# cocowy1/Cost-Volume-Aggregation-in-Stereo-Matching-Revisited

Measured on AMD Instinct MI355X. Metric: cost-volumes/sec (fwd+bwd) at 544x960 D=192, higher is better.
Workload: dtype f32

## Files before the change

### cost-volume-aggregation-in-stereo-matching-revisited_amd/csrc/conv3d_wgrad_f16x2.hip

```cpp
#include "dca_frag.h"
#include "dca_tiles.h"
#include <type_traits>

namespace {

constexpr int NT = 2;
constexpr int TD = 2, TH = 4, TW = 16;
constexpr int NROW = TD * TH;
constexpr int NGRP = 2, NACC = 7;
static_assert(NROW / NGRP == TH, "a K-step group is one d plane of the tile");
constexpr int HD = TD + 2, HH = TH + 2, NHROW = HD * HH;
constexpr int XV = TW + 2;
constexpr int VB = 64;
constexpr int X_TERM = NHROW * XV * VB;
constexpr int Y_TERM = NROW * TW * VB;
constexpr int X_OFF = 0, Y_OFF = NT * X_TERM;
constexpr int IMG_BYTES = Y_OFF + NT * Y_TERM;
constexpr int LDS_BYTES = 2 * IMG_BYTES;
static_assert(LDS_BYTES >= 4 * 7 * 4096 && LDS_BYTES + 128 <= 160 * 1024, "LDS");
constexpr int NXW = NT * NHROW * XV * 4, KXW = (NXW + 511) / 512;
constexpr int NYW = NT * NROW * TW * 4, KYW = NYW / 512;
constexpr int NXQ = NHROW * 4 * 4, NXE = NHROW * 2 * 4, NYQ = NROW * 4 * 4;
static_assert(NXQ + NYQ == 512 && NYW % 512 == 0, "staging items");

struct WX2Args {
  const float* x;
  const float* dy;
  float* part;
  int N, Cx, Cy, D, H, W;
  int nTD, nTH, nTW, nCxT;
  const int* xexps;
  const int* yexps;
};

template <bool XP, bool YP>
__global__ __launch_bounds__(512) void wgrad3_f16x2_kernel(WX2Args a) {
  extern __shared__ __attribute__((aligned(16))) char smem[];
  const int tid = threadIdx.x, lane = tid & 63, wv = tid >> 6, l31 = lane & 31, half = lane >> 5;
  const int grp = wv >> 2, wq = wv & 3;
  const int ct = blockIdx.y, cy0 = (ct / a.nCxT) * 32, cx0 = (ct % a.nCxT) * 32;

  const DcaTileWalk walk = dca_my_tile_walk((long)a.N * a.nTD * a.nTH * a.nTW);
  const int t_begin = walk.begin, t_end = walk.end, t_step = walk.step;

  f32x16 acc[NACC];
#pragma unroll
  for (int j = 0; j < NACC; ++j)
#pragma unroll
    for (int r = 0; r < 16; ++r) acc[j][r] = 0.f;

  const int cstride = a.D * a.H * a.W;
  const long xsample = (long)a.Cx * cstride, ysample = (long)a.Cy * cstride;

  const int lane_off = (8 * half + ((lane & 15) >> 2)) * VB + (16 * ((lane >> 4) & 1) + 4 * (lane & 3)) * 2;

  float4 pw[(XP ? KXW : 0) + (YP ? KYW : 0) + ((XP || YP) ? 0 : 1)];
  float4 rq[(XP && YP) ? 1 : 8];
  float re[XP ? 1 : 8];
  int ex8[(XP && YP) ? 1 : 8];
  if constexpr (!XP || !YP) {
    const bool isy = !YP && (XP || tid >= NXQ);
#pragma unroll
    for (int j = 0; j < 8; ++j) {
      const int c = (isy ? cy0 : cx0) + (tid & 3) * 8 + j;
      ex8[j] = (c < (isy ? a.Cy : a.Cx)) ? dca_coherent_loadi((isy ? a.yexps : a.xexps) + c) : 0;
    }
  }
  int xcrd[XP ? KXW : 1], ycrd[YP ? KYW : 1];
  if constexpr (XP) {
#pragma unroll
    for (int k = 0; k < KXW; ++k) {
      const int it = tid + 512 * k, cg = it & 3, vv = it >> 2, v = vv % XV, r = vv / XV, hrow = r % NHROW, term = r / NHROW;
      xcrd[k] = (it < NXW) ? ((hrow / HH) | ((hrow % HH) << 4) | (v << 8) | (term << 16) | (cg << 20)) : -1;
    }
  }
  if constexpr (YP) {
#pragma unroll
    for (int k = 0; k < KYW; ++k) {
      const int it = tid + 512 * k, cg = it & 3, vv = it >> 2, v = vv % TW, r = vv / TW, row = r % NROW, term = r / NROW;
      ycrd[k] = (row / TH) | ((row % TH) << 4) | (v << 8) | (term << 16) | (cg << 20);
    }
  }
  auto decode = [&](int tile, int& n, int& d0, int& h0, int& w0) __attribute__((always_inline)) {
    dca_tile_decode<TD, TH, TW>(tile, a.nTD, a.nTH, a.nTW, n, d0, h0, w0);
  };
  auto load_tile = [&](int n, int d0, int h0, int w0, int part = -1) __attribute__((always_inline)) {
    const __amdgpu_buffer_rsrc_t xr = dca_rsrc(a.x + (long)n * xsample, xsample * 4);
    const __amdgpu_buffer_rsrc_t yr = dca_rsrc(a.dy + (long)n * ysample, ysample * 4);
    if constexpr (XP) {
#pragma unroll
      for (int k = 0; k < KXW; ++k) {
        if ((part == 0 && k >= 4) || (part == 1 && k < 4)) continue;
        int crd = xcrd[k];
        asm volatile("" : "+v"(crd));
        const int d = d0 - 1 + (crd & 15), h = h0 - 1 + ((crd >> 4) & 15), w = w0 - 1 + ((crd >> 8) & 255);
        const int term = (crd >> 16) & 1, g = (cx0 >> 3) + ((crd >> 20) & 3);
        const int ok = (int)(crd >= 0) & (int)(g * 8 < a.Cx) & (int)((unsigned)d < (unsigned)a.D) &
                       (int)((unsigned)h < (unsigned)a.H) & (int)((unsigned)w < (unsigned)a.W);
        pw[k] = dca_bload4(xr, term * (a.Cx * cstride * 2) + (g * cstride + (d * a.H + h) * a.W + w) * 16, ok);
      }
    } else {
      if (part != 1 && tid < NXQ) {
        const int cg = tid & 3, quad = (tid >> 2) & 3, hrow = tid >> 4;
        const int d = d0 - 1 + hrow / HH, h = h0 - 1 + hrow % HH, w = w0 + 4 * quad, c0 = cx0 + cg * 8;
        const int ok = (int)((unsigned)d < (unsigned)a.D) & (int)((unsigned)h < (unsigned)a.H) & (int)(w + 3 < a.W);
        const int off = (c0 * cstride + (d * a.H + h) * a.W + w) * 4;
#pragma unroll
        for (int j = 0; j < 8; ++j) rq[j] = dca_bload4(xr, off + j * cstride * 4, ok & (int)(c0 + j < a.Cx));
      }
      if (part != 0 && tid < NXE) {
        const int cg = tid & 3, side = (tid >> 2) & 1, hrow = tid >> 3;
        const int d = d0 - 1 + hrow / HH, h = h0 - 1 + hrow % HH, w = side ? w0 + TW : w0 - 1, c0 = cx0 + cg * 8;
        const int ok = (int)((unsigned)d < (unsigned)a.D) & (int)((unsigned)h < (unsigned)a.H) & (int)((unsigned)w < (unsigned)a.W);
        const int off = (c0 * cstride + (d * a.H + h) * a.W + w) * 4;
#pragma unroll
        for (int j = 0; j < 8; ++j) re[j] = dca_bload1(xr, off + j * cstride * 4, ok & (int)(c0 + j < a.Cx));
      }
    }
    if (part == 0) return;
    if constexpr (YP) {
#pragma unroll
      for (int k = 0; k < KYW; ++k) {
        int crd = ycrd[k];
        asm volatile("" : "+v"(crd));
        const int d = d0 + (crd & 15), h = h0 + ((crd >> 4) & 15), w = w0 + ((crd >> 8) & 255);
        const int term = (crd >> 16) & 1, g = (cy0 >> 3) + ((crd >> 20) & 3);
        const int ok = (int)(g * 8 < a.Cy) & (int)(d < a.D) & (int)(h < a.H) & (int)(w < a.W);
        pw[(XP ? KXW : 0) + k] = dca_bload4(yr, term * (a.Cy * cstride * 2) + (g * cstride + (d * a.H + h) * a.W + w) * 16, ok);
      }
    } else {
      if (XP || tid >= NXQ) {
        const int u = XP ? tid : tid - NXQ;
        if (u < NYQ) {
          const int cg = u & 3, quad = (u >> 2) & 3, row = u >> 4;
          const int d = d0 + row / TH, h = h0 + row % TH, w = w0 + 4 * quad, c0 = cy0 + cg * 8;
          const int ok = (int)(d < a.D) & (int)(h < a.H) & (int)(w + 3 < a.W);
          const int off = (c0 * cstride + (d * a.H + h) * a.W + w) * 4;
#pragma unroll
          for (int j = 0; j < 8; ++j) rq[j] = dca_bload4(yr, off + j * cstride * 4, ok & (int)(c0 + j < a.Cy));
        }
      }
    }
  };
  typedef __attribute__((address_space(3))) char lds_char;
  const int wvu = __builtin_amdgcn_readfirstlane(tid >> 6);
  const unsigned lds0 = (unsigned)(unsigned long)(lds_char*)smem;
  auto desc = [&](const void* base, long bytes) __attribute__((always_inline)) {
    const unsigned long long b = (unsigned long long)base;
    u32x4 r;
    r.x = __builtin_amdgcn_readfirstlane((unsigned)b);
    r.y = __builtin_amdgcn_readfirstlane((unsigned)(b >> 32)) & 0xffffu;
    r.z = __builtin_amdgcn_readfirstlane((unsigned)bytes);
    r.w = 0x00020000u;
    return r;
  };
  auto glds16 = [&](u32x4 rs, int voff, unsigned lds_byte) __attribute__((always_inline)) {
    unsigned keep;
    asm volatile("s_mov_b32 %0, m0\n\ts_mov_b32 m0, %2\n\ts_nop 0\n\tbuffer_load_dwordx4 %1, %3, 0 offen lds\n\ts_mov_b32 m0, %0"
                 : "=&s"(keep) : "v"(voff), "s"(lds_byte), "s"(rs) : "memory");
  };
  auto glds_tile = [&](int n, int d0, int h0, int w0, int part, int buf) __attribute__((always_inline)) {
    if constexpr (XP && YP) {
      const u32x4 xr = desc(a.x + (long)n * xsample, xsample * 4), yr = desc(a.dy + (long)n * ysample, ysample * 4);
      const unsigned img = lds0 + buf * IMG_BYTES;
#pragma unroll
      for (int k = 0; k < KXW; ++k) {
        if ((part == 0 && k >= 4) || (part == 1 && k < 4)) continue;
        if (512 * k + 64 * wvu < NXW) {
          int crd = xcrd[k];
          asm volatile("" : "+v"(crd));
          const int d = d0 - 1 + (crd & 15), h = h0 - 1 + ((crd >> 4) & 15), w = w0 - 1 + ((crd >> 8) & 255);
          const int term = (crd >> 16) & 1, g = (cx0 >> 3) + ((crd >> 20) & 3);
          const int ok = (int)(g * 8 < a.Cx) & (int)((unsigned)d < (unsigned)a.D) & (int)((unsigned)h < (unsigned)a.H) &
                         (int)((unsigned)w < (unsigned)a.W);
          glds16(xr, dca_pred_off(term * (a.Cx * cstride * 2) + (g * cstride + (d * a.H + h) * a.W + w) * 16, ok),
                 img + X_OFF + (512 * k + 64 * wvu) * 16);
        }
      }
      if (part == 0) return;
#pragma unroll
      for (int k = 0; k < KYW; ++k) {
        int crd = ycrd[k];
        asm volatile("" : "+v"(crd));
        const int d = d0 + (crd & 15), h = h0 + ((crd >> 4) & 15), w = w0 + ((crd >> 8) & 255);
        const int term = (crd >> 16) & 1, g = (cy0 >> 3) + ((crd >> 20) & 3);
        const int ok = (int)(g * 8 < a.Cy) & (int)(d < a.D) & (int)(h < a.H) & (int)(w < a.W);
        glds16(yr, dca_pred_off(term * (a.Cy * cstride * 2) + (g * cstride + (d * a.H + h) * a.W + w) * 16, ok),
               img + Y_OFF + (512 * k + 64 * wvu) * 16);
      }
    }
  };

  auto split_word = [&](const float (&v)[8], char* dst, int term_stride) __attribute__((always_inline)) {
    f16x8 hv, lv;
#pragma unroll
    for (int j = 0; j < 8; ++j) {
      _Float16 h, l;
      x2_split(v[j], ex8[j], h, l);
      hv[j] = h; lv[j] = l;
    }
    *(f16x8*)dst = hv;
    *(f16x8*)(dst + term_stride) = lv;
  };
  auto quad_words = [&](char* dst, int term_stride) __attribute__((always_inline)) {
    const float* q0 = (const float*)&rq[0];
#pragma unroll
    for (int vv = 0; vv < 4; ++vv) {
      const float v[8] = {q0[vv], q0[4 + vv], q0[8 + vv], q0[12 + vv], q0[16 + vv], q0[20 + vv], q0[24 + vv], q0[28 + vv]};
      split_word(v, dst + vv * VB, term_stride);
    }
  };
  auto store_tile = [&]() __attribute__((always_inline)) {
    if constexpr (XP) {
#pragma unroll
      for (int k = 0; k < KXW; ++k) {
        const int it = tid + 512 * k;
        if (it < NXW) *(float4*)(smem + X_OFF + it * 16) = pw[k];
      }
    } else {
      if (tid < NXQ) {
        const int cg = tid & 3, quad = (tid >> 2) & 3, hrow = tid >> 4;
        quad_words(smem + X_OFF + (hrow * XV + 1 + 4 * quad) * VB + cg * 16, X_TERM);
      }
      if (tid < NXE) {
        const int cg = tid & 3, side = (tid >> 2) & 1, hrow = tid >> 3;
        const float v[8] = {re[0], re[1], re[2], re[3], re[4], re[5], re[6], re[7]};
        split_word(v, smem + X_OFF + (hrow * XV + (side ? XV - 1 : 0)) * VB + cg * 16, X_TERM);
      }
    }
    if constexpr (YP) {
#pragma unroll
      for (int k = 0; k < KYW; ++k) *(float4*)(smem + Y_OFF + (tid + 512 * k) * 16) = pw[(XP ? KXW : 0) + k];
    } else {
      if (XP || tid >= NXQ) {
        const int u = XP ? tid : tid - NXQ;
        if (u < NYQ) {
          const int cg = u & 3, quad = (u >> 2) & 3, row = u >> 4;
          quad_words(smem + Y_OFF + (row * TW + 4 * quad) * VB + cg * 16, Y_TERM);
        }
      }
    }
  };

  auto mfma_tile = [&](auto WQC, bool more, int next_tile, int buf) __attribute__((always_inline)) {
    constexpr int WQ = decltype(WQC)::value;
    constexpr int TAP0 = 7 * WQ, TAP1 = (TAP0 + 7 < 27) ? TAP0 + 7 : 27, NTAP = TAP1 - TAP0;
#pragma unroll 1
    for (int i = 0; i < TH; ++i) {
      if ((i == 1 || i == 2) && more) {
        int nn, nd0, nh0, nw0;
        decode(next_tile, nn, nd0, nh0, nw0);
        if constexpr (XP && YP) glds_tile(nn, nd0, nh0, nw0, i - 1, buf ^ 1);
        else load_tile(nn, nd0, nh0, nw0, i - 1);
      }
      const char* yb = smem + buf * IMG_BYTES + Y_OFF + ((grp * TH + i) * TW) * VB + lane_off;
      const char* xb = smem + buf * IMG_BYTES + X_OFF + ((grp * HH + i) * XV) * VB + lane_off;
      f16x8 ay[NT];
#pragma unroll
      for (int term = 0; term < NT; ++term) ay[term] = tr_frag(yb + term * Y_TERM, 4 * VB);
      f16x8 bx[2][NT];
      auto load_b = [&](int tap, int slot) __attribute__((always_inline)) {
        const int kd = tap / 9, kh = (tap / 3) % 3, kw = tap % 3;
#pragma unroll
        for (int term = 0; term < NT; ++term) bx[slot][term] = tr_frag(xb + term * X_TERM + ((kd * HH + kh) * XV + kw) * VB, 4 * VB);
      };
      load_b(TAP0, 0);
#pragma unroll
      for (int j = 0; j < NTAP; ++j) {
        const int cur = j & 1;
        if (j + 1 < NTAP) load_b(TAP0 + j + 1, cur ^ 1);
        acc[j] = __builtin_amdgcn_mfma_f32_32x32x16_f16(ay[0], bx[cur][1], acc[j], 0, 0, 0);
        acc[j] = __builtin_amdgcn_mfma_f32_32x32x16_f16(ay[1], bx[cur][0], acc[j], 0, 0, 0);
        acc[j] = __builtin_amdgcn_mfma_f32_32x32x16_f16(ay[0], bx[cur][0], acc[j], 0, 0, 0);
        if (j + 1 < NTAP) {
          __builtin_amdgcn_sched_group_barrier(0x100, 2, 0);
          __builtin_amdgcn_sched_group_barrier(0x008, 1, 0);
          __builtin_amdgcn_sched_group_barrier(0x100, 2, 0);
          __builtin_amdgcn_sched_group_barrier(0x008, 2, 0);
        }
        __builtin_amdgcn_sched_barrier(0);
      }
    }
  };

  if (t_begin < t_end) {
    int n, d0, h0, w0;
    decode(t_begin, n, d0, h0, w0);
    if constexpr (XP && YP) {
      glds_tile(n, d0, h0, w0, -1, 0);
      __builtin_amdgcn_s_waitcnt(0x0f70);
    } else {
      load_tile(n, d0, h0, w0);
      store_tile();
    }
    __syncthreads();
    int buf = 0;
#pragma unroll 1
    for (int tile = t_begin; tile < t_end; tile += t_step) {
      const bool more = tile + t_step < t_end;
      switch (wq) {
        case 0: mfma_tile(std::integral_constant<int, 0>{}, more, tile + t_step, buf); break;
        case 1: mfma_tile(std::integral_constant<int, 1>{}, more, tile + t_step, buf); break;
        case 2: mfma_tile(std::integral_constant<int, 2>{}, more, tile + t_step, buf); break;
        default: mfma_tile(std::integral_constant<int, 3>{}, more, tile + t_step, buf); break;
      }
      if constexpr (XP && YP) __builtin_amdgcn_s_waitcnt(0x0f70);
      __syncthreads();
      if constexpr (XP && YP) {
        buf ^= 1;
      } else {
        if (more) store_tile();
        __syncthreads();
      }
    }
  }

  __syncthreads();
  int* ey_lds = (int*)(smem + LDS_BYTES);
  if (tid < 32) ey_lds[tid] = (cy0 + tid < a.Cy) ? dca_coherent_loadi(a.yexps + cy0 + tid) : 0;
  __syncthreads();
  const int xe_l = (cx0 + l31 < a.Cx) ? dca_coherent_loadi(a.xexps + cx0 + l31) : 0;
  int ninv[16];
#pragma unroll
  for (int r = 0; r < 16; ++r) ninv[r] = -(ey_lds[(r & 3) + 8 * (r >> 2) + 4 * half] + xe_l);
  float* red = (float*)smem;
  if (grp == 1) {
#pragma unroll
    for (int j = 0; j < 7; ++j)
#pragma unroll
      for (int r = 0; r < 16; ++r)
        red[((wq * 7 + j) * 32 + (r & 3) + 8 * (r >> 2) + 4 * half) * 32 + l31] = acc[j][r];
  }
  __syncthreads();
  if (grp == 0) {
    float* slab = a.part + ((long)blockIdx.x * gridDim.y + ct) * 27 * 1024;
#pragma unroll
    for (int j = 0; j < 7; ++j) {
      const int tap = 7 * wq + j;
      if (tap < 27) {
#pragma unroll
        for (int r = 0; r < 16; ++r) {
          const int co = (r & 3) + 8 * (r >> 2) + 4 * half;
          slab[tap * 1024 + co * 32 + l31] = ldexpf(acc[j][r] + red[((wq * 7 + j) * 32 + co) * 32 + l31], ninv[r]);
        }
      }
    }
  }
}

}

extern "C" long dca_conv3d_wgrad_x2_workspace(int N, int Cx, int Cy, int D, int H, int W) {
  if (N <= 0 || Cx <= 0 || Cy <= 0 || D <= 0 || H <= 0 || W <= 0) return 0;
  return dca_wgrad_split_geometry<TD, TH, TW>(N, Cx, Cy, D, H, W).part_floats;
}

extern "C" int dca_conv3d_wgrad_x2(const void* x, int x_packed, const int* xexps, const void* dy, int dy_packed,
                                   const int* yexps, float* part, float* dw, int N, int Cx, int Cy, int D, int H, int W,
                                   long s_cy, long s_cx, hipStream_t stream) {
  DCA_REQUIRE(x && dy && part && dw && xexps && yexps && N > 0 && Cx > 0 && Cy > 0 && D > 0 && H > 0 && W > 0);
  DCA_REQUIRE(((((uintptr_t)x | (uintptr_t)dy) & 15) == 0));
  DCA_REQUIRE((x_packed ? Cx % 8 == 0 : W % 4 == 0) && (dy_packed ? Cy % 8 == 0 : W % 4 == 0));
  DCA_REQUIRE((long)Cx * D * H * W * 4 < 0x7ffffff0L && (long)Cy * D * H * W * 4 < 0x7ffffff0L);
  WX2Args a;
  a.x = (const float*)x; a.dy = (const float*)dy; a.part = part; a.xexps = xexps; a.yexps = yexps;
  a.N = N; a.Cx = Cx; a.Cy = Cy; a.D = D; a.H = H; a.W = W;
  const DcaWgradSplitGeom g = dca_wgrad_split_geometry<TD, TH, TW>(N, Cx, Cy, D, H, W);
  a.nTD = g.t.nTD; a.nTH = g.t.nTH; a.nTW = g.t.nTW; a.nCxT = g.nCxT;
  DCA_REQUIRE(g.t.fits() && g.nCT <= 65535);
  const int lds = LDS_BYTES + 128;
  auto kern = x_packed ? (dy_packed ? wgrad3_f16x2_kernel<true, true> : wgrad3_f16x2_kernel<true, false>)
                       : (dy_packed ? wgrad3_f16x2_kernel<false, true> : wgrad3_f16x2_kernel<false, false>);
  hipError_t e = hipFuncSetAttribute((const void*)kern, hipFuncAttributeMaxDynamicSharedMemorySize, lds);
  if (e != hipSuccess) return (int)e;
  hipLaunchKernelGGL(kern, dim3(g.nblk, g.nCT), dim3(512), lds, stream, a);
  int st = dca_launch_status();
  if (st) return st;
  return dca_internal_wgrad_reduce(part, dw, g.nblk, g.nCxT, g.nCT, 27, Cy, Cx, s_cy, s_cx, stream);
}
```

### cost-volume-aggregation-in-stereo-matching-revisited_amd/ops.py

```python
from __future__ import annotations

import ctypes
import os
import threading

import torch

from ._call import _C, _L, _chk, _ptr, _raw_device, _raw_stream, _req, _req_no_grad, _stream, _vp
from .guided import GUIDE, guide_params, hints_to_quarter


def _opt(t, name):
    return None if t is None else _req(t, name)


class _GwcVolume(torch.autograd.Function):
    @staticmethod
    def forward(ctx, ref, tgt, maxdisp, num_groups):
        ref, tgt = _req(ref, "build_gwc_volume"), _req(tgt, "build_gwc_volume")
        B, C, H, W = ref.shape
        vol = torch.empty((B, num_groups, maxdisp, H, W), device=ref.device, dtype=torch.float32)
        with torch.cuda.device_of(ref):
            _chk(_L().dca_gwc_volume_fwd(_ptr(ref), _ptr(tgt), _ptr(vol), B, C, H, W, maxdisp, num_groups, _stream()),
                 "dca_gwc_volume_fwd")
# ... 242 lines not shown
        _chk(_L().dca_softargmin_stats(_ptr(x), _ptr(out), B, K, HW, min(radius, K), _stream()), "dca_softargmin_stats")
    return out


class _UpSoftArgmin(torch.autograd.Function):

    @staticmethod
    def forward(ctx, logits, scale):
        logits = _req(logits, "up_softargmin")
        B, n, hc, wc = logits.shape
        disp = torch.empty((B, 1, scale * hc, scale * wc), device=logits.device, dtype=torch.float32)
        with torch.cuda.device_of(logits):
            _chk(_L().dca_up_softargmin_fwd(_ptr(logits), _ptr(disp), B, n, hc, wc, scale, _stream()),
                 "dca_up_softargmin_fwd")
        ctx.save_for_backward(logits)
        ctx.scale = scale
        return disp

    @staticmethod
    def backward(ctx, g):
        (logits,) = ctx.saved_tensors
        g = _req(g, "up_softargmin.backward")
        B, n, hc, wc = logits.shape
        s = ctx.scale
        g1 = torch.empty((B, n, s * hc, s * wc), device=logits.device, dtype=torch.float32)
        gl = torch.empty_like(logits)
        with torch.cuda.device_of(logits):
            _chk(_L().dca_up_softargmin_bwd(_ptr(logits), _ptr(g), _ptr(g1), _ptr(gl), B, n, hc, wc, s, _stream()),
                 "dca_up_softargmin_bwd")
        return gl, None


def up_softargmin(logits, scale):
    if logits.shape[1] > 64 or logits.shape[1] < 2 or scale not in (2, 4, 8):
        return softargmin(trilinear_upsample(logits.unsqueeze(1), scale).squeeze(1))
    return _UpSoftArgmin.apply(logits, int(scale))


def _round_up(a, m):
    return (a + m - 1) // m * m


_CONV_MODE = os.environ.get("DCA_CONV", "x2")
CONV_X3 = _CONV_MODE != "fp32"
CONV_X2 = _CONV_MODE == "x2"
WGRAD_S2_X2 = os.environ.get("DCA_WGRAD_S2", "x2") != "fp32"
DECONV_X3 = os.environ.get("DCA_DECONV", "x3") != "fp32"
C1_WGRAD_FUSED = os.environ.get("DCA_C1_WGRAD", "fused") != "expand"
CONV_S2_X2 = os.environ.get("DCA_CONV_S2", "x2") != "fp32"
BN_FUSE = os.environ.get("DCA_BN_FUSE", "1") != "0"
C1_BWD_FUSE = os.environ.get("DCA_C1_BWD", "fused") != "split"
SKIP_FOLD = os.environ.get("DCA_SKIP_FOLD", "1") != "0"
C1_HEAD_BWD = os.environ.get("DCA_C1_HEAD_BWD", "fused") != "split"
_X3_MIN_WORKGROUPS = 1


AMAX_STATS = {"tagged": 0, "computed": 0, "packed": 0}
CSLOTS = _C["DCA_AMAX_CSLOTS"]
AMAX_EMIT = os.environ.get("DCA_AMAX_EMIT", "1") != "0"
PACK = os.environ.get("DCA_PACK", "1") != "0"


def _cslots(C, device):
    if not AMAX_EMIT:
        return None
    return torch.empty((C * CSLOTS,), device=device, dtype=torch.int32)


def _ver(t):
    return None if t.is_inference() else t._version


def _tag_cmax(t, slots, nslots):
    if slots is not None:
        t._dca_cmax = (slots, int(nslots), _ver(t))
    return t


def _tag_px2(t, exps):
    t._dca_px2 = (exps,)
    return t


def _tag_exps(t, exps):
    t._dca_exps = (exps, _ver(t))


def _tag_twin(t, twin):
    t._dca_twin = (twin, _ver(t))


def _tag_ok(t, name):
    tag = getattr(t, name, None)
    if tag is not None and tag[-1] == _ver(t) and tag[0].device == t.device:
        return tag
    return None


def _copy_tags(src, dst):
    cmax, exps, twin = _tag_ok(src, "_dca_cmax"), _tag_ok(src, "_dca_exps"), _tag_ok(src, "_dca_twin")
    if cmax is not None:
        _tag_cmax(dst, cmax[0], cmax[1])
    if exps is not None:
        _tag_exps(dst, exps[0])
    if twin is not None:
        _tag_twin(dst, twin[0])
# ... 149 lines not shown
    if not (training and pack_dy and float(slope) == 0.0) or has_pre or has_post:
        return "split"
    if tuple(weight.shape) != (1, 32, 3, 3, 3) or h.dim() != 5 or h.shape[1] != 32 or h.shape[-1] % 4:
        return "split"
    if not all(t.is_cuda and t.dtype == torch.float32 and t.requires_grad for t in (h, weight)):
        return "split"
    if _is_packed(h) or h.data_ptr() % 16 or not h.is_contiguous() or h[0].numel() * 4 >= 0x7ffffff0:
        return "split"
    return "fused"


class _SkipBn:
    __slots__ = ("y", "part", "bn", "into")

    def __init__(self, y, part, bn, into):
        self.y, self.part, self.bn, self.into = y, part, bn, into


def _skip_fold_route(x, conv_b, bn_b, slope_b, bn_out):
    if not (SKIP_FOLD and PACK and CONV_X2 and bn_out is not None and torch.is_grad_enabled() and _lp_dtype() is None):
        return "apply"
    C = bn_b.num_features
    if not (bn_b.training and bn_out.training) or bn_out.num_features != C or C % 8 or float(slope_b) != 1.0:
        return "apply"
    if x.dtype != torch.float32 or bn_b.weight is None or bn_b.bias is None:
        return "apply"
    return "fold" if _c1_bwd_route(x, None, conv_b.weight) == "fused" else "apply"


def _k3s1(weight, stride, transposed, x2, head=False):
    return x2 is None and not transposed and int(stride) == 1 and weight.shape[2] == 3 and (weight.shape[0] == 1) == head


def _x2_pairs(xp, yp, W):
    return W % 4 == 0 or (xp and yp)


def _wgrad_family(x, dy, Cx, Cy, ksize, stride):
    Di, Hi, Wi = x.shape[2:]
    Do, Ho, Wo = dy.shape[2:]
    xp, yp = _is_packed(x), _is_packed(dy)
    split = (CONV_X3 and ksize == 3 and x.data_ptr() % 16 == 0 and dy.data_ptr() % 16 == 0
             and max(Cx, Cy) * Di * Hi * Wi * 4 < 0x7ffffff0)
    if split and CONV_X2 and stride == 1 and _x2_pairs(xp, yp, Wi):
        return "x2"
    if xp or yp:
        raise RuntimeError("weight gradient: a packed px2 operand can only feed the f16x2 3x3x3 stride-1 kernel")
    if split and stride == 1 and Wi % 4 == 0:
        return "x3"
    if (split and CONV_X2 and WGRAD_S2_X2 and stride == 2 and Wi % 4 == 0 and Wo % 4 == 0
            and (Do, Ho, Wo) == ((Di + 1) // 2, (Hi + 1) // 2, (Wi + 1) // 2)):
        return "s2x2"
    return "mfma"


def _slice_width(ksize, stride, transposed, B):
    if ksize == 1 or transposed:
        return 32
    return 32 if (stride == 1 and B <= 32) else 64


def _prep_weight(w_src, A, B, K, src_ab, flip, ksize, stride, transposed, b_off=0, Bn=None):
    Bn = B if Bn is None else Bn
    if ksize == 1:
        Apad = 32 if A <= 32 else 64
        Bpad = 32
    else:
        Apad = _round_up(A, 8)
        Bpad = 32 if (transposed or (stride == 1 and Bn <= 32)) else 64
    def build():
        wt = torch.empty((K, Apad, Bpad), device=w_src.device, dtype=torch.float32)
        _chk(_L().dca_conv3d_prep_weight(_ptr(w_src), _ptr(wt), A, Bn, Apad, Bpad, K, int(src_ab), int(flip), B, b_off,
                                         _stream()), "dca_conv3d_prep_weight")
        return wt
    return _memo(("prep", A, B, K, int(src_ab), int(flip), Apad, Bpad, b_off, Bn), (w_src,), build,
                 (0, A, Bn, Apad, Bpad, K, int(src_ab), int(flip), B, b_off)), Apad


def _x2_weights(prefix, x, w_src, A, B, src_ab, flip, cached_key):
    lib = _L()
    wx = torch.empty((getattr(lib, prefix + "_weight_bytes")(A, B) // 2,), device=x.device, dtype=torch.int16)
    xexps = _exps_cached(x)
    if xexps is not None:
        AMAX_STATS[cached_key] += 1
        slots, nslots = None, 0
    else:
        slots, nslots = _slots_of(x)
        xexps = torch.empty((A,), device=x.device, dtype=torch.int32)
    _chk(getattr(lib, prefix + "_prep_weight")(_ptr(w_src), _ptr(wx), A, B, int(src_ab), int(flip), _ptr(slots), nslots,
                                               _ptr(xexps), _stream()), prefix + "_prep_weight")
    if slots is not None:
        _tag_exps(x, xexps)
    return wx, xexps


def _x3_weights(w_src, A, B, src_ab, flip):
    def build():
        w3 = torch.empty((_L().dca_conv3d_x3_weight_bytes(A, B) // 2,), device=w_src.device, dtype=torch.int16)
        _chk(_L().dca_conv3d_x3_prep_weight(_ptr(w_src), _ptr(w3), A, B, int(src_ab), int(flip), _stream()),
             "dca_conv3d_x3_prep_weight")
        return w3
    return _memo(("x3prep", A, B, int(src_ab), int(flip)), (w_src,), build, (1, A, B, 0, 0, 27, int(src_ab), int(flip), B, 0))


def _out_dims(dims, ksize, stride, transposed):
    if ksize == 1 or stride == 1:
# ... 75 lines not shown
                                                    S, _stream()), "dca_conv1_x3_forward_stats")
            else:
                _chk(lib.dca_conv1_x3_forward(_ptr(x), _ptr(x2), _ptr(wf), _ptr(y), _ptr(scale), _ptr(shift),
                                              _ptr(res_pre), _ptr(res_post), float(slope), N, C1, C2, bn, B, b0, S,
                                              _stream()), "dca_conv1_x3_forward")
    else:
        width = _slice_width(ksize, stride, transposed, B)
        for b0 in range(0, B, width):
            bn = min(width, B - b0)
            wt, Apad = _prep_weight(w_src, A, B, K, src_ab, flip, ksize, stride, transposed, b0, bn)
            _chk(lib.dca_conv3d_forward(_ptr(x), _ptr(x2), _ptr(wt), _ptr(y), _ptr(scale), _ptr(shift), _ptr(res_pre),
                                        _ptr(res_post), float(slope), N, A, C1, bn, Apad, B, b0, Di, Hi, Wi, Do, Ho, Wo,
                                        ksize, stride, int(transposed), _stream()), "dca_conv3d_forward")
    return (y, part) if want_stats else y


def conv3d_prepared(x, wt, A, Apad, B, ksize, stride, transposed):
    N = x.shape[0]
    Di, Hi, Wi = x.shape[2:]
    Do, Ho, Wo = _out_dims((Di, Hi, Wi), ksize, stride, transposed)
    y = torch.empty((N, B, Do, Ho, Wo), device=x.device, dtype=torch.float32)
    _chk(_L().dca_conv3d_forward(_ptr(x), None, _ptr(wt), _ptr(y), None, None, None, None, 1.0, N, A, A, B, Apad, B, 0,
                                 Di, Hi, Wi, Do, Ho, Wo, ksize, stride, int(transposed), _stream()),
         "dca_conv3d_forward")
    return y


def _conv_forward_impl(x, x2, weight, stride, transposed, scale=None, shift=None, slope=1.0, res_pre=None,
                       res_post=None, want_stats=False, emit_amax=False):
    ksize = weight.shape[2]
    K = ksize ** 3
    if transposed:
        Cin, Cout = weight.shape[0], weight.shape[1]
        src_ab = 1
    else:
        Cout, Cin = weight.shape[0], weight.shape[1]
        src_ab = 0
    assert x.shape[1] + (x2.shape[1] if x2 is not None else 0) == Cin, "conv3d: channel mismatch"
    return _conv_sliced(x, x2, weight, Cin, Cout, K, src_ab, 0, ksize, stride, transposed, scale, shift, slope,
                        res_pre, res_post, want_stats, emit_amax)


def _wgrad(x, dy, dw_view_ptr_tensor, dst_offset, Cx, Cy, ksize, stride, s_cy, s_cx):
    N = x.shape[0]
    Di, Hi, Wi = x.shape[2:]
    Do, Ho, Wo = dy.shape[2:]
    dst = _vp(dw_view_ptr_tensor.data_ptr() + 4 * dst_offset)
    lib = _L()
    family = _wgrad_family(x, dy, Cx, Cy, ksize, stride)
    workspace = lambda nws: torch.empty((nws,), device=x.device, dtype=torch.float32)
    if family == "x2":
        xex, yex = _exps_of(x), _exps_of(dy)
        part = workspace(lib.dca_conv3d_wgrad_x2_workspace(N, Cx, Cy, Di, Hi, Wi))
        _chk(lib.dca_conv3d_wgrad_x2(_ptr(x), int(_is_packed(x)), _ptr(xex), _ptr(dy), int(_is_packed(dy)), _ptr(yex),
                                     _ptr(part), dst, N, Cx, Cy, Di, Hi, Wi, s_cy, s_cx, _stream()), "dca_conv3d_wgrad_x2")
    elif family == "x3":
        part = workspace(lib.dca_conv3d_wgrad_x3_workspace(N, Cx, Cy, Di, Hi, Wi))
        _chk(lib.dca_conv3d_wgrad_x3(_ptr(x), _ptr(dy), _ptr(part), dst, N, Cx, Cy, Di, Hi, Wi, s_cy, s_cx, _stream()),
             "dca_conv3d_wgrad_x3")
    elif family == "s2x2":
        xex, yex = _exps_of(x), _exps_of(dy)
        part = workspace(lib.dca_conv3d_wgrad_s2_x2_workspace(N, Cx, Cy, Di, Hi, Wi))
        _chk(lib.dca_conv3d_wgrad_s2_x2(_ptr(x), _ptr(xex), _ptr(dy), _ptr(yex), _ptr(part), dst, N, Cx, Cy, Di, Hi, Wi,
                                        s_cy, s_cx, _stream()), "dca_conv3d_wgrad_s2_x2")
    else:
        part = workspace(lib.dca_conv3d_wgrad_workspace(N, Cx, Cy, Do, Ho, Wo, ksize, stride))
        _chk(lib.dca_conv3d_wgrad(_ptr(x), _ptr(dy), _ptr(part), dst, N, Cx, Cy, Di, Hi, Wi, Do, Ho, Wo, ksize, stride,
                                  s_cy, s_cx, _stream()), "dca_conv3d_wgrad")


class _Conv3dC1(torch.autograd.Function):

    @staticmethod
    def forward(ctx, x, weight, head_fused=False):
        x, weight = _req(x, "conv3d"), _req(weight, "conv3d.weight")
        ctx.head_fused = bool(head_fused)
        N, C, D, H, W = x.shape
        with torch.cuda.device_of(x):
            T = _conv_sliced(x, None, weight, C, 27, 1, 1, 0, 1, 1, False)
            y = torch.empty((N, 1, D, H, W), device=x.device, dtype=torch.float32)
            _chk(_L().dca_conv3d_c1_gather(_ptr(T), _ptr(y), N, D, H, W, _stream()), "dca_conv3d_c1_gather")
        ctx.save_for_backward(x, weight)
        return y

    @staticmethod
    def backward(ctx, dy):
        x, weight = ctx.saved_tensors
        dy = _req(dy, "conv3d.backward")
        N, C, D, H, W = x.shape
        gx = gw = None
        lib = _L()
        with torch.cuda.device_of(x):
            if ctx.head_fused:
                gx = dy.expand(N, C, D, H, W)
                gx._dca_head = (dy, weight)
            elif ctx.needs_input_grad[0]:
                gx = torch.empty_like(x)
                _chk(lib.dca_conv3d_c1_bwd_data(_ptr(dy), _ptr(weight), _ptr(gx), N, C, D, H, W, _stream()),
                     "dca_conv3d_c1_bwd_data")
            if ctx.needs_input_grad[1]:
                gw = torch.empty_like(weight)
                if (C1_WGRAD_FUSED and W % 4 == 0 and x.data_ptr() % 16 == 0 and dy.data_ptr() % 16 == 0
                        and x.numel() * 4 < 0x7ffffff0):
                    nws = lib.dca_conv3d_wgrad_workspace(N, C, 27, D, H, W, 1, 1)
                    part = torch.empty((nws,), device=x.device, dtype=torch.float32)
                    _chk(lib.dca_conv3d_c1_wgrad(_ptr(x), _ptr(dy), _ptr(part), _ptr(gw), N, C, D, H, W, _stream()),
                         "dca_conv3d_c1_wgrad")
                else:
# ... 1098 lines not shown
```

### include/dca_hip.h

```cpp
#ifndef DCA_HIP_H
#define DCA_HIP_H

#include <hip/hip_runtime_api.h>

#ifdef __cplusplus
extern "C" {
#endif

#define DCA_ABI_VERSION 21
int dca_abi_version(void);

#define DCA_BF16 1
#define DCA_FP16 2

int dca_gwc_volume_fwd(const float* ref, const float* tgt, float* vol, int B, int C, int H, int W, int maxdisp,
                       int num_groups, hipStream_t stream);
int dca_gwc_volume_bwd(const float* gvol, const float* ref, const float* tgt, float* gref, float* gtgt, int B, int C,
                       int H, int W, int maxdisp, int num_groups, hipStream_t stream);
long dca_gwc_volume_bwd_rows(int B, int C, int H, int W, int maxdisp, int num_groups);
int dca_concat_volume_fwd(const float* ref, const float* tgt, float* vol, int B, int C, int H, int W, int maxdisp,
                          hipStream_t stream);
int dca_concat_volume_bwd(const float* gvol, float* gref, float* gtgt, int B, int C, int H, int W, int maxdisp,
                          hipStream_t stream);

// ... 39 lines not shown
int dca_conv3d_x3_prep_weight(const float* w, void* wx, int A, int B, int src_ab, int flip, hipStream_t stream);
int dca_conv3d_x3_forward(const float* x, const void* wx, float* y, const float* scale, const float* shift,
                          const float* res_pre, const float* res_post, float slope, int N, int Cin, int Cout, int D,
                          int H, int W, hipStream_t stream);

int dca_deconv3d_x3_forward(const float* x, const void* wx, float* y, const float* scale, const float* shift,
                            const float* res_pre, const float* res_post, float slope, int N, int Cin, int Cout, int Di,
                            int Hi, int Wi, hipStream_t stream);

long dca_conv3d_x3_stats_chunks(int N, int Cout, int D, int H, int W);
int dca_conv3d_x3_forward_stats(const float* x, const void* wx, float* y, double* stat_part, int N, int Cin, int Cout,
                                int D, int H, int W, hipStream_t stream);
long dca_conv1_x3_stats_chunks(int N, long S);
int dca_conv1_x3_forward_stats(const float* x, const float* x2, const void* wfrag, float* y, double* stat_part, int N,
                               int C1, int C2, int Cout, int CoutTotal, int co_off, long S, hipStream_t stream);
long dca_deconv3d_x3_stats_chunks(int N, int Di, int Hi, int Wi);
int dca_deconv3d_x3_forward_stats(const float* x, const void* wx, float* y, double* stat_part, int N, int Cin, int Cout,
                                  int Di, int Hi, int Wi, hipStream_t stream);
int dca_bn_finalize_centered(const double* part, int nchunk, const float* gamma, const float* beta, float* running_mean,
                             float* running_var, float momentum, float eps, float* stats, int* zexps,
                             const unsigned* rpre_slots, int rpre_n, const unsigned* rpost_slots, int rpost_n, int C,
                             hipStream_t stream);

long dca_conv3d_wgrad_x3_workspace(int N, int Cx, int Cy, int D, int H, int W);
int dca_conv3d_wgrad_x3(const float* x, const float* dy, float* part, float* dw, int N, int Cx, int Cy, int D, int H,
                        int W, long s_cy, long s_cx, hipStream_t stream);

#define DCA_AMAX_CSLOTS 1024
int dca_cmax_f32(const float* x, int N, int C, long S, unsigned* slots, hipStream_t stream);
int dca_cmax_exps(const unsigned* slots, int nslots, int C, int* exps, hipStream_t stream);
long dca_conv3d_x2_weight_bytes(int Cin, int Cout);
int dca_conv3d_x2_prep_weight(const float* w, void* wx, int A, int B, int src_ab, int flip, const unsigned* x_slots,
                              int nslots, int* xexps, hipStream_t stream);
int dca_conv3d_x2_forward(const void* x, int packed, const int* xexps, const void* wx, float* y, const float* scale,
                          const float* shift, const float* res_pre, const float* res_post, float slope, unsigned* y_cmax,
                          int N, int Cin, int Cout, int D, int H, int W, hipStream_t stream);
long dca_conv3d_x2_stats_chunks(int N, int Cout, int D, int H, int W);
int dca_conv3d_x2_forward_stats(const void* x, int packed, const int* xexps, const void* wx, float* y, double* stat_part,
                                int N, int Cin, int Cout, int D, int H, int W, hipStream_t stream);
long dca_conv3d_wgrad_s2_x2_workspace(int N, int Cx, int Cy, int D, int H, int W);
int dca_conv3d_wgrad_s2_x2(const float* f, const int* f_exps, const float* c, const int* c_exps, float* part,
                           float* dw, int N, int Cx, int Cy, int D, int H, int W, long s_cy, long s_cx, hipStream_t stream);
long dca_conv3d_s2x2_weight_bytes(int Cin, int Cout);
int dca_conv3d_s2x2_prep_weight(const float* w, void* wx, int A, int B, int src_ab, int flip, const unsigned* x_slots,
                                int nslots, int* xexps, hipStream_t stream);
long dca_conv3d_s2x2_out_slots(int N, int Cout, int Di, int Hi, int Wi);
int dca_conv3d_s2x2_forward(const float* x, const int* xexps, const void* wx, float* y, const float* scale, const float* shift,
                            float slope, const float* res_post, unsigned* y_cmax, int N, int Cin, int Cout, int Di, int Hi, int Wi,
                            hipStream_t stream);
long dca_conv3d_wgrad_x2_workspace(int N, int Cx, int Cy, int D, int H, int W);
int dca_conv3d_wgrad_x2(const void* x, int x_packed, const int* xexps, const void* dy, int dy_packed, const int* yexps,
                        float* part, float* dw, int N, int Cx, int Cy, int D, int H, int W, long s_cy, long s_cx,
                        hipStream_t stream);

int dca_conv3d_c1_gather(const float* T, float* y, int N, int D, int H, int W, hipStream_t stream);
int dca_conv3d_c1_wgrad(const float* x, const float* dy, float* part, float* dw, int N, int C, int D, int H, int W,
                        hipStream_t stream);
int dca_conv3d_c1_expand(const float* dy, float* G, int N, int D, int H, int W, hipStream_t stream);
int dca_conv3d_c1_bwd_data(const float* dy, const float* w, float* dx, int N, int C, int D, int H, int W,
                           hipStream_t stream);

int dca_bn_num_chunks(int C, long S);
int dca_bn_pack_chunks(int C, long S);
int dca_bn_stats(const float* x, double* part, int N, int C, long S, hipStream_t stream);
int dca_bn_finalize(const double* part, int nchunk, double count, const float* gamma, const float* beta,
                    float* running_mean, float* running_var, float momentum, float eps, int training, float* stats,
                    int* zexps, const unsigned* rpre_slots, int rpre_n, const unsigned* rpost_slots, int rpost_n, int C,
                    hipStream_t stream);
int dca_bn_apply(const float* y, const float* stats, const float* res_pre, const float* res_post, float* z, int N,
                 int C, long S, float slope, unsigned* zmax, unsigned* ymax, hipStream_t stream);
int dca_bn_apply_pack(const float* y, const float* stats, const int* zexps, void* zp, int N, int C, long S, float slope,
                      unsigned* ymax, const float* res_pre, const float* res_post, float* zf, unsigned* zmax,
                      hipStream_t stream);
int dca_bn_backward(const float* dz, const float* y, const float* res_pre, const float* stats, double* part,
                    float* dgb, float* dy, float* g_out, int N, int C, long S, float slope, int training,
                    unsigned* dmax, hipStream_t stream);
int dca_bn_backward_reduce(const float* dz, const float* y, const float* stats, double* part, float* dgb, int N, int C,
                           long S, float slope, int training, hipStream_t stream);
int dca_bn_backward_pack(const float* dz, const float* y, const float* stats, double* part, float* dgb, void* dyp,
                         int* dyexps, unsigned* gmax, const unsigned* ymax, int ymax_slots, int N, int C, long S,
                         float slope, int training, hipStream_t stream);
int dca_bn_backward_pack_c1_chunks(int N, int D, int H, int W);
int dca_bn_backward_pack_c1_grid(int N, int D, int H, int W);
int dca_bn_backward_pack_c1(const float* dlogit, const float* w_head, const float* y, const float* stats, double* part,
                            float* dgb, void* dyp, int* dyexps, unsigned* gmax, const unsigned* ymax, int ymax_slots, int N,
                            int C, int D, int H, int W, float slope, int training, hipStream_t stream);
int dca_bn_skip_max(const float* y_r, const float* stats_r, int N, int C, long S, unsigned* slots, hipStream_t stream);
int dca_bn_apply_pack_skip(const float* y, const float* stats, const int* zexps, void* zp, int N, int C, long S, float slope,
                           unsigned* ymax, const float* y_r, const float* stats_r, const float* res_post, float* zf,
                           unsigned* zmax, hipStream_t stream);
int dca_bn_backward_skip(const float* dz, const float* y, const float* y_r, const float* stats, const float* stats_r,
                         double* part, double* part_r, float* dgb, float* dgb_r, float* dy, float* g_out, int N, int C,
                         long S, float slope, int training, unsigned* dmax, hipStream_t stream);

int dca_avgpool3d_fwd(const float* x, float* y, long NC, int Di, int Hi, int Wi, hipStream_t stream);
int dca_avgpool3d_bwd(const float* gy, float* gx, const float* res, const float* res2, long NC, int Di, int Hi, int Wi,
                     hipStream_t stream);

int dca_trilinear_fwd(const float* x, float* y, long NC, int Di, int Hi, int Wi, int scale, hipStream_t stream);
int dca_trilinear_bwd(const float* gy, float* gx, long NC, int Di, int Hi, int Wi, int scale, hipStream_t stream);

int dca_context_inject_fwd(const float* x, const float* preds, float* key, int* kstar, float* e, float* pm,
                           float* denom, float* part, int B, int C, int n, long HW, hipStream_t stream);
int dca_context_inject_bwd(const float* dkey, const float* x, const float* preds, const int* kstar, const float* e,
                           const float* pm, const float* denom, float* dx, float* dpreds, float* dw, float* T,
                           float* part, int B, int C, int n, long HW, hipStream_t stream);
// ... 285 lines not shown
```

Before: 41.56.

## Stack multiple conv taps into MFMA K-dimension for partial Cx channel tiles

When the input-channel count leaves a tail tile of 8 or 16 real channels, the wgrad kernel now packs several 3x3x3 taps into one 32-wide MFMA operand instead of padding the tile with zero channels. Per-lane tap offsets index the halo in LDS, so each wave issues fewer MFMA groups for the tail tile, and the epilogue scatters results back to the correct tap and channel. A padded entry point and an environment switch keep the old path available. This adds kernel instantiations and a separate tail code path with its own staging and scheduling, which raises compile size and the risk of indexing errors.

```diff
diff --git a/cost-volume-aggregation-in-stereo-matching-revisited_amd/csrc/conv3d_wgrad_f16x2.hip b/cost-volume-aggregation-in-stereo-matching-revisited_amd/csrc/conv3d_wgrad_f16x2.hip
--- a/cost-volume-aggregation-in-stereo-matching-revisited_amd/csrc/conv3d_wgrad_f16x2.hip
+++ b/cost-volume-aggregation-in-stereo-matching-revisited_amd/csrc/conv3d_wgrad_f16x2.hip
@@ -33,12 +33,15 @@
   const int* yexps;
 };
 
-template <bool XP, bool YP>
+template <bool XP, bool YP, int R>
 __global__ __launch_bounds__(512) void wgrad3_f16x2_kernel(WX2Args a) {
+  static_assert(R == 0 || R == 8 || R == 16, "tap stacking needs r | 32 real channels");
+  constexpr int S = R ? 32 / R : 1, NG = (27 + S - 1) / S, NGW = (NG + 3) / 4, TSH = R == 16 ? 1 : 0;
   extern __shared__ __attribute__((aligned(16))) char smem[];
   const int tid = threadIdx.x, lane = tid & 63, wv = tid >> 6, l31 = lane & 31, half = lane >> 5;
   const int grp = wv >> 2, wq = wv & 3;
   const int ct = blockIdx.y, cy0 = (ct / a.nCxT) * 32, cx0 = (ct % a.nCxT) * 32;
+  const bool tail = R != 0 && a.Cx - cx0 == R;
 
   const DcaTileWalk walk = dca_my_tile_walk((long)a.N * a.nTD * a.nTH * a.nTW);
   const int t_begin = walk.begin, t_end = walk.end, t_step = walk.step;
@@ -52,7 +55,18 @@
   const int cstride = a.D * a.H * a.W;
   const long xsample = (long)a.Cx * cstride, ysample = (long)a.Cy * cstride;
 
-  const int lane_off = (8 * half + ((lane & 15) >> 2)) * VB + (16 * ((lane >> 4) & 1) + 4 * (lane & 3)) * 2;
+  const int lane_row = 16 * ((lane >> 4) & 1) + 4 * (lane & 3);
+  const int lane_off = (8 * half + ((lane & 15) >> 2)) * VB + lane_row * 2;
+  const int lane_off_x = R ? (8 * half + ((lane & 15) >> 2)) * VB + (lane_row % (R ? R : 1)) * 2 : lane_off;
+  int toff[R ? NGW : 1];
+  if constexpr (R != 0) {
+#pragma unroll
+    for (int k = 0; k < NGW; ++k) {
+      int tap = ((NGW * wq + k) * S + lane_row / R);
+      tap = tap < 26 ? tap : 26;
+      toff[k] = (((tap / 9) * HH + (tap / 3) % 3) * XV + tap % 3) * VB;
+    }
+  }
 
   float4 pw[(XP ? KXW : 0) + (YP ? KYW : 0) + ((XP || YP) ? 0 : 1)];
   float4 rq[(XP && YP) ? 1 : 8];
@@ -62,7 +76,7 @@
     const bool isy = !YP && (XP || tid >= NXQ);
 #pragma unroll
     for (int j = 0; j < 8; ++j) {
-      const int c = (isy ? cy0 : cx0) + (tid & 3) * 8 + j;
+      const int c = (isy ? cy0 + (tid & 3) * 8 : cx0 + (tail ? tid & ((1 << TSH) - 1) : tid & 3) * 8) + j;
       ex8[j] = (c < (isy ? a.Cy : a.Cx)) ? dca_coherent_loadi((isy ? a.yexps : a.xexps) + c) : 0;
     }
   }
@@ -84,7 +98,8 @@
   auto decode = [&](int tile, int& n, int& d0, int& h0, int& w0) __attribute__((always_inline)) {
     dca_tile_decode<TD, TH, TW>(tile, a.nTD, a.nTH, a.nTW, n, d0, h0, w0);
   };
-  auto load_tile = [&](int n, int d0, int h0, int w0, int part = -1) __attribute__((always_inline)) {
+  auto load_tile = [&](auto TLC, int n, int d0, int h0, int w0, int part = -1) __attribute__((always_inline)) {
+    constexpr int SH = decltype(TLC)::value ? TSH : 2;
     const __amdgpu_buffer_rsrc_t xr = dca_rsrc(a.x + (long)n * xsample, xsample * 4);
     const __amdgpu_buffer_rsrc_t yr = dca_rsrc(a.dy + (long)n * ysample, ysample * 4);
     if constexpr (XP) {
@@ -100,16 +115,16 @@
         pw[k] = dca_bload4(xr, term * (a.Cx * cstride * 2) + (g * cstride + (d * a.H + h) * a.W + w) * 16, ok);
       }
     } else {
-      if (part != 1 && tid < NXQ) {
-        const int cg = tid & 3, quad = (tid >> 2) & 3, hrow = tid >> 4;
+      if (part != 1 && tid < ((NHROW * 4) << SH)) {
+        const int cg = tid & ((1 << SH) - 1), quad = (tid >> SH) & 3, hrow = tid >> (SH + 2);
         const int d = d0 - 1 + hrow / HH, h = h0 - 1 + hrow % HH, w = w0 + 4 * quad, c0 = cx0 + cg * 8;
         const int ok = (int)((unsigned)d < (unsigned)a.D) & (int)((unsigned)h < (unsigned)a.H) & (int)(w + 3 < a.W);
         const int off = (c0 * cstride + (d * a.H + h) * a.W + w) * 4;
 #pragma unroll
         for (int j = 0; j < 8; ++j) rq[j] = dca_bload4(xr, off + j * cstride * 4, ok & (int)(c0 + j < a.Cx));
       }
-      if (part != 0 && tid < NXE) {
-        const int cg = tid & 3, side = (tid >> 2) & 1, hrow = tid >> 3;
+      if (part != 0 && tid < ((NHROW * 2) << SH)) {
+        const int cg = tid & ((1 << SH) - 1), side = (tid >> SH) & 1, hrow = tid >> (SH + 1);
         const int d = d0 - 1 + hrow / HH, h = h0 - 1 + hrow % HH, w = side ? w0 + TW : w0 - 1, c0 = cx0 + cg * 8;
         const int ok = (int)((unsigned)d < (unsigned)a.D) & (int)((unsigned)h < (unsigned)a.H) & (int)((unsigned)w < (unsigned)a.W);
         const int off = (c0 * cstride + (d * a.H + h) * a.W + w) * 4;
@@ -210,7 +225,8 @@
       split_word(v, dst + vv * VB, term_stride);
     }
   };
-  auto store_tile = [&]() __attribute__((always_inline)) {
+  auto store_tile = [&](auto TLC) __attribute__((always_inline)) {
+    constexpr int SH = decltype(TLC)::value ? TSH : 2;
     if constexpr (XP) {
 #pragma unroll
       for (int k = 0; k < KXW; ++k) {
@@ -218,12 +234,12 @@
         if (it < NXW) *(float4*)(smem + X_OFF + it * 16) = pw[k];
       }
     } else {
-      if (tid < NXQ) {
-        const int cg = tid & 3, quad = (tid >> 2) & 3, hrow = tid >> 4;
+      if (tid < ((NHROW * 4) << SH)) {
+        const int cg = tid & ((1 << SH) - 1), quad = (tid >> SH) & 3, hrow = tid >> (SH + 2);
         quad_words(smem + X_OFF + (hrow * XV + 1 + 4 * quad) * VB + cg * 16, X_TERM);
       }
-      if (tid < NXE) {
-        const int cg = tid & 3, side = (tid >> 2) & 1, hrow = tid >> 3;
+      if (tid < ((NHROW * 2) << SH)) {
+        const int cg = tid & ((1 << SH) - 1), side = (tid >> SH) & 1, hrow = tid >> (SH + 1);
         const float v[8] = {re[0], re[1], re[2], re[3], re[4], re[5], re[6], re[7]};
         split_word(v, smem + X_OFF + (hrow * XV + (side ? XV - 1 : 0)) * VB + cg * 16, X_TERM);
       }
@@ -251,7 +267,7 @@
         int nn, nd0, nh0, nw0;
         decode(next_tile, nn, nd0, nh0, nw0);
         if constexpr (XP && YP) glds_tile(nn, nd0, nh0, nw0, i - 1, buf ^ 1);
-        else load_tile(nn, nd0, nh0, nw0, i - 1);
+        else load_tile(std::false_type{}, nn, nd0, nh0, nw0, i - 1);
       }
       const char* yb = smem + buf * IMG_BYTES + Y_OFF + ((grp * TH + i) * TW) * VB + lane_off;
       const char* xb = smem + buf * IMG_BYTES + X_OFF + ((grp * HH + i) * XV) * VB + lane_off;
@@ -283,6 +299,46 @@
     }
   };
 
+  auto mfma_tail = [&](auto, bool more, int next_tile, int buf) __attribute__((always_inline)) {
+#pragma unroll 1
+    for (int i = 0; i < TH; ++i) {
+      if ((i == 1 || i == 2) && more) {
+        int nn, nd0, nh0, nw0;
+        decode(next_tile, nn, nd0, nh0, nw0);
+        if constexpr (XP && YP) glds_tile(nn, nd0, nh0, nw0, i - 1, buf ^ 1);
+        else load_tile(std::true_type{}, nn, nd0, nh0, nw0, i - 1);
+      }
+      const char* yb = smem + buf * IMG_BYTES + Y_OFF + ((grp * TH + i) * TW) * VB + lane_off;
+      const char* xb = smem + buf * IMG_BYTES + X_OFF + ((grp * HH + i) * XV) * VB + lane_off_x;
+      f16x8 ay[NT];
+#pragma unroll
+      for (int term = 0; term < NT; ++term) ay[term] = tr_frag(yb + term * Y_TERM, 4 * VB);
+      f16x8 bx[2][NT];
+      auto load_b = [&](int k, int slot) __attribute__((always_inline)) {
+#pragma unroll
+        for (int term = 0; term < NT; ++term) bx[slot][term] = tr_frag(xb + toff[k] + term * X_TERM, 4 * VB);
+      };
+      load_b(0, 0);
+#pragma unroll
+      for (int k = 0; k < NGW; ++k) {
+        const int cur = k & 1;
+        if (k + 1 < NGW) load_b(k + 1, cur ^ 1);
+        acc[k] = __builtin_amdgcn_mfma_f32_32x32x16_f16(ay[0], bx[cur][1], acc[k], 0, 0, 0);
+        acc[k] = __builtin_amdgcn_mfma_f32_32x32x16_f16(ay[1], bx[cur][0], acc[k], 0, 0, 0);
+        acc[k] = __builtin_amdgcn_mfma_f32_32x32x16_f16(ay[0], bx[cur][0], acc[k], 0, 0, 0);
+        if (k + 1 < NGW) {
+          __builtin_amdgcn_sched_group_barrier(0x100, 2, 0);
+          __builtin_amdgcn_sched_group_barrier(0x008, 1, 0);
+          __builtin_amdgcn_sched_group_barrier(0x100, 2, 0);
+          __builtin_amdgcn_sched_group_barrier(0x008, 2, 0);
+        }
+        __builtin_amdgcn_sched_barrier(0);
+      }
+    }
+  };
+
+  auto run = [&](auto TLC) __attribute__((always_inline)) {
+    constexpr bool TL = decltype(TLC)::value;
   if (t_begin < t_end) {
     int n, d0, h0, w0;
     decode(t_begin, n, d0, h0, w0);
@@ -290,15 +346,16 @@
       glds_tile(n, d0, h0, w0, -1, 0);
       __builtin_amdgcn_s_waitcnt(0x0f70);
     } else {
-      load_tile(n, d0, h0, w0);
-      store_tile();
+      load_tile(TLC, n, d0, h0, w0);
+      store_tile(TLC);
     }
     __syncthreads();
     int buf = 0;
 #pragma unroll 1
     for (int tile = t_begin; tile < t_end; tile += t_step) {
       const bool more = tile + t_step < t_end;
-      switch (wq) {
+      if constexpr (TL) mfma_tail(TLC, more, tile + t_step, buf);
+      else switch (wq) {
         case 0: mfma_tile(std::integral_constant<int, 0>{}, more, tile + t_step, buf); break;
         case 1: mfma_tile(std::integral_constant<int, 1>{}, more, tile + t_step, buf); break;
         case 2: mfma_tile(std::integral_constant<int, 2>{}, more, tile + t_step, buf); break;
@@ -309,17 +366,25 @@
       if constexpr (XP && YP) {
         buf ^= 1;
       } else {
-        if (more) store_tile();
+        if (more) store_tile(TLC);
         __syncthreads();
       }
     }
+  }
+  };
+  if constexpr (R != 0) {
+    if (tail) run(std::true_type{});
+    else run(std::false_type{});
+  } else {
+    run(std::false_type{});
   }
 
   __syncthreads();
   int* ey_lds = (int*)(smem + LDS_BYTES);
   if (tid < 32) ey_lds[tid] = (cy0 + tid < a.Cy) ? dca_coherent_loadi(a.yexps + cy0 + tid) : 0;
   __syncthreads();
-  const int xe_l = (cx0 + l31 < a.Cx) ? dca_coherent_loadi(a.xexps + cx0 + l31) : 0;
+  const int cil = tail ? l31 % (R ? R : 1) : l31;
+  const int xe_l = (cx0 + cil < a.Cx) ? dca_coherent_loadi(a.xexps + cx0 + cil) : 0;
   int ninv[16];
 #pragma unroll
   for (int r = 0; r < 16; ++r) ninv[r] = -(ey_lds[(r & 3) + 8 * (r >> 2) + 4 * half] + xe_l);
@@ -334,6 +399,20 @@
   __syncthreads();
   if (grp == 0) {
     float* slab = a.part + ((long)blockIdx.x * gridDim.y + ct) * 27 * 1024;
+    if (tail) {
+#pragma unroll
+      for (int j = 0; j < (R ? NGW : 0); ++j) {
+        const int tap = (NGW * wq + j) * S + l31 / (R ? R : 1);
+        if (tap < 27) {
+#pragma unroll
+          for (int r = 0; r < 16; ++r) {
+            const int co = (r & 3) + 8 * (r >> 2) + 4 * half;
+            slab[tap * 1024 + co * 32 + cil] = ldexpf(acc[j][r] + red[((wq * 7 + j) * 32 + co) * 32 + l31], ninv[r]);
+          }
+        }
+      }
+      return;
+    }
 #pragma unroll
     for (int j = 0; j < 7; ++j) {
       const int tap = 7 * wq + j;
@@ -355,13 +434,15 @@
   return dca_wgrad_split_geometry<TD, TH, TW>(N, Cx, Cy, D, H, W).part_floats;
 }
 
-extern "C" int dca_conv3d_wgrad_x2(const void* x, int x_packed, const int* xexps, const void* dy, int dy_packed,
-                                   const int* yexps, float* part, float* dw, int N, int Cx, int Cy, int D, int H, int W,
-                                   long s_cy, long s_cx, hipStream_t stream) {
+template <int R>
+static int wgrad_x2_launch(const void* x, int x_packed, const int* xexps, const void* dy, int dy_packed, const int* yexps,
+                           float* part, float* dw, int N, int Cx, int Cy, int D, int H, int W, long s_cy, long s_cx,
+                           hipStream_t stream) {
   DCA_REQUIRE(x && dy && part && dw && xexps && yexps && N > 0 && Cx > 0 && Cy > 0 && D > 0 && H > 0 && W > 0);
   DCA_REQUIRE(((((uintptr_t)x | (uintptr_t)dy) & 15) == 0));
   DCA_REQUIRE((x_packed ? Cx % 8 == 0 : W % 4 == 0) && (dy_packed ? Cy % 8 == 0 : W % 4 == 0));
   DCA_REQUIRE((long)Cx * D * H * W * 4 < 0x7ffffff0L && (long)Cy * D * H * W * 4 < 0x7ffffff0L);
+  DCA_REQUIRE(R == 0 || Cx % 32 == R);
   WX2Args a;
   a.x = (const float*)x; a.dy = (const float*)dy; a.part = part; a.xexps = xexps; a.yexps = yexps;
   a.N = N; a.Cx = Cx; a.Cy = Cy; a.D = D; a.H = H; a.W = W;
@@ -369,8 +450,8 @@
   a.nTD = g.t.nTD; a.nTH = g.t.nTH; a.nTW = g.t.nTW; a.nCxT = g.nCxT;
   DCA_REQUIRE(g.t.fits() && g.nCT <= 65535);
   const int lds = LDS_BYTES + 128;
-  auto kern = x_packed ? (dy_packed ? wgrad3_f16x2_kernel<true, true> : wgrad3_f16x2_kernel<true, false>)
-                       : (dy_packed ? wgrad3_f16x2_kernel<false, true> : wgrad3_f16x2_kernel<false, false>);
+  auto kern = x_packed ? (dy_packed ? wgrad3_f16x2_kernel<true, true, R> : wgrad3_f16x2_kernel<true, false, R>)
+                       : (dy_packed ? wgrad3_f16x2_kernel<false, true, R> : wgrad3_f16x2_kernel<false, false, R>);
   hipError_t e = hipFuncSetAttribute((const void*)kern, hipFuncAttributeMaxDynamicSharedMemorySize, lds);
   if (e != hipSuccess) return (int)e;
   hipLaunchKernelGGL(kern, dim3(g.nblk, g.nCT), dim3(512), lds, stream, a);
@@ -378,3 +459,19 @@
   if (st) return st;
   return dca_internal_wgrad_reduce(part, dw, g.nblk, g.nCxT, g.nCT, 27, Cy, Cx, s_cy, s_cx, stream);
 }
+
+extern "C" int dca_conv3d_wgrad_x2(const void* x, int x_packed, const int* xexps, const void* dy, int dy_packed,
+                                   const int* yexps, float* part, float* dw, int N, int Cx, int Cy, int D, int H, int W,
+                                   long s_cy, long s_cx, hipStream_t stream) {
+  if (Cx % 32 == 8)
+    return wgrad_x2_launch<8>(x, x_packed, xexps, dy, dy_packed, yexps, part, dw, N, Cx, Cy, D, H, W, s_cy, s_cx, stream);
+  if (Cx % 32 == 16)
+    return wgrad_x2_launch<16>(x, x_packed, xexps, dy, dy_packed, yexps, part, dw, N, Cx, Cy, D, H, W, s_cy, s_cx, stream);
+  return wgrad_x2_launch<0>(x, x_packed, xexps, dy, dy_packed, yexps, part, dw, N, Cx, Cy, D, H, W, s_cy, s_cx, stream);
+}
+
+extern "C" int dca_conv3d_wgrad_x2_padded(const void* x, int x_packed, const int* xexps, const void* dy, int dy_packed,
+                                          const int* yexps, float* part, float* dw, int N, int Cx, int Cy, int D, int H,
+                                          int W, long s_cy, long s_cx, hipStream_t stream) {
+  return wgrad_x2_launch<0>(x, x_packed, xexps, dy, dy_packed, yexps, part, dw, N, Cx, Cy, D, H, W, s_cy, s_cx, stream);
+}
diff --git a/cost-volume-aggregation-in-stereo-matching-revisited_amd/ops.py b/cost-volume-aggregation-in-stereo-matching-revisited_amd/ops.py
--- a/cost-volume-aggregation-in-stereo-matching-revisited_amd/ops.py
+++ b/cost-volume-aggregation-in-stereo-matching-revisited_amd/ops.py
@@ -318,6 +318,7 @@
 C1_BWD_FUSE = os.environ.get("DCA_C1_BWD", "fused") != "split"
 SKIP_FOLD = os.environ.get("DCA_SKIP_FOLD", "1") != "0"
 C1_HEAD_BWD = os.environ.get("DCA_C1_HEAD_BWD", "fused") != "split"
+WGRAD_TAIL_STACK = os.environ.get("DCA_WGRAD_TAIL", "stack") != "pad"
 _X3_MIN_WORKGROUPS = 1
 
 
@@ -573,6 +574,12 @@
             and (Do, Ho, Wo) == ((Di + 1) // 2, (Hi + 1) // 2, (Wi + 1) // 2)):
         return "s2x2"
     return "mfma"
+
+
+def _wgrad_tail_route(Cx):
+    if Cx % 32 not in (8, 16):
+        return "none"
+    return "stack" if WGRAD_TAIL_STACK else "pad"
 
 
 def _slice_width(ksize, stride, transposed, B):
@@ -754,8 +761,9 @@
     if family == "x2":
         xex, yex = _exps_of(x), _exps_of(dy)
         part = workspace(lib.dca_conv3d_wgrad_x2_workspace(N, Cx, Cy, Di, Hi, Wi))
-        _chk(lib.dca_conv3d_wgrad_x2(_ptr(x), int(_is_packed(x)), _ptr(xex), _ptr(dy), int(_is_packed(dy)), _ptr(yex),
-                                     _ptr(part), dst, N, Cx, Cy, Di, Hi, Wi, s_cy, s_cx, _stream()), "dca_conv3d_wgrad_x2")
+        entry = "dca_conv3d_wgrad_x2_padded" if _wgrad_tail_route(Cx) == "pad" else "dca_conv3d_wgrad_x2"
+        _chk(getattr(lib, entry)(_ptr(x), int(_is_packed(x)), _ptr(xex), _ptr(dy), int(_is_packed(dy)), _ptr(yex),
+                                 _ptr(part), dst, N, Cx, Cy, Di, Hi, Wi, s_cy, s_cx, _stream()), entry)
     elif family == "x3":
         part = workspace(lib.dca_conv3d_wgrad_x3_workspace(N, Cx, Cy, Di, Hi, Wi))
         _chk(lib.dca_conv3d_wgrad_x3(_ptr(x), _ptr(dy), _ptr(part), dst, N, Cx, Cy, Di, Hi, Wi, s_cy, s_cx, _stream()),
diff --git a/include/dca_hip.h b/include/dca_hip.h
--- a/include/dca_hip.h
+++ b/include/dca_hip.h
@@ -115,6 +115,9 @@
 int dca_conv3d_wgrad_x2(const void* x, int x_packed, const int* xexps, const void* dy, int dy_packed, const int* yexps,
                         float* part, float* dw, int N, int Cx, int Cy, int D, int H, int W, long s_cy, long s_cx,
                         hipStream_t stream);
+int dca_conv3d_wgrad_x2_padded(const void* x, int x_packed, const int* xexps, const void* dy, int dy_packed,
+                               const int* yexps, float* part, float* dw, int N, int Cx, int Cy, int D, int H, int W,
+                               long s_cy, long s_cx, hipStream_t stream);
 
 int dca_conv3d_c1_gather(const float* T, float* y, int N, int D, int H, int W, hipStream_t stream);
 int dca_conv3d_c1_wgrad(const float* x, const float* dy, float* part, float* dw, int N, int C, int D, int H, int W,
```

New measurement: 41.51. Within noise of the previous version (-0.1%).
